# yhsong0804/P-NTFields

Measured on AMD Instinct MI355X. Metric: (start,goal) tau+grad-tau evals/sec at batch=1M, Gibson 3D, higher is better.
Workload: dtype f32; 1 GPU; gibson_multi_env_tau_grad (C3/C4 shape: 1048576 pairs/GPU, 10 envs, per-pair env id, dim 3); pairs_per_gpu=1048576, global_batch=1048576, envs=10, grad_mode=exact, allgather_outputs=False, parallelism=dp1, rccl_world_size=1

## Files before the change

p-ntfields_amd/csrc/pntf_wide.h:

```cpp
#pragma once
#include "pntf_field.h"
#include "pntf_stamp.h"

namespace pntf {

typedef float f32x16 __attribute__((ext_vector_type(16)));

__device__ __forceinline__ f32x16 mfma32(float a, float b, f32x16 c) {
  return __builtin_amdgcn_mfma_f32_32x32x2f32(a, b, c, 0, 0, 0);
}
__device__ __forceinline__ f32x16 zero16() {
  f32x16 z;
#pragma unroll
  for (int r = 0; r < 16; ++r) z[r] = 0.f;
  return z;
}

constexpr int WNL = 6;
typedef __bf16 wbf16x8 __attribute__((ext_vector_type(8)));
typedef __bf16 wbf16x2 __attribute__((ext_vector_type(2)));
typedef float wf32x2 __attribute__((ext_vector_type(2)));
__device__ __forceinline__ void wx6_split(const f32x16& v, int b, wbf16x8 (&s)[3]) {
#pragma unroll
  for (int i = 0; i < 4; ++i) {
    wf32x2 x = {v[8 * b + 2 * i], v[8 * b + 2 * i + 1]};
    const wbf16x2 p0 = __builtin_convertvector(x, wbf16x2);
#ifdef PNTF_ABL_NOSPLIT
    s[0][2 * i] = s[1][2 * i] = s[2][2 * i] = p0[0];
    s[0][2 * i + 1] = s[1][2 * i + 1] = s[2][2 * i + 1] = p0[1];
    continue;
#endif
#if PNTF_X6_DOT
    const wf32x2 r1 = x6_resid(x, p0);
    const wbf16x2 p1 = __builtin_convertvector(r1, wbf16x2);
    const wf32x2 r2 = x6_resid(r1, p1);
#else
    const wf32x2 r1 = x - __builtin_convertvector(p0, wf32x2);
    const wbf16x2 p1 = __builtin_convertvector(r1, wbf16x2);
    const wf32x2 r2 = r1 - __builtin_convertvector(p1, wf32x2);
#endif
    const wbf16x2 p2 = __builtin_convertvector(r2, wbf16x2);
    s[0][2 * i] = p0[0]; s[0][2 * i + 1] = p0[1];
    s[1][2 * i] = p1[0]; s[1][2 * i + 1] = p1[1];
    s[2][2 * i] = p2[0]; s[2][2 * i + 1] = p2[1];
  }
}
__device__ __forceinline__ f32x16 wx6_mma(const f32x4& w0, const f32x4& w1, const f32x4& w2,
                                          const wbf16x8 (&x)[3], f32x16 acc) {
  const wbf16x8 a0 = __builtin_bit_cast(wbf16x8, w0), a1 = __builtin_bit_cast(wbf16x8, w1),
                a2 = __builtin_bit_cast(wbf16x8, w2);
  acc = __builtin_amdgcn_mfma_f32_32x32x16_bf16(a2, x[0], acc, 0, 0, 0);
  acc = __builtin_amdgcn_mfma_f32_32x32x16_bf16(a1, x[1], acc, 0, 0, 0);
  acc = __builtin_amdgcn_mfma_f32_32x32x16_bf16(a0, x[2], acc, 0, 0, 0);
  acc = __builtin_amdgcn_mfma_f32_32x32x16_bf16(a1, x[0], acc, 0, 0, 0);
  acc = __builtin_amdgcn_mfma_f32_32x32x16_bf16(a0, x[1], acc, 0, 0, 0);
  return __builtin_amdgcn_mfma_f32_32x32x16_bf16(a0, x[0], acc, 0, 0, 0);
}
constexpr float WKAPPA = WIDE_KAPPA;
constexpr float WKAPPA_INV = 0.0693147180559945309f;
__device__ __forceinline__ SpSig wsp_sig(float y) {
#ifdef PNTF_ABL_CHEAPACT
  return SpSig{fmaxf(y, 0.f) * 0.5f + 0.01f, 0.5f};
#endif
  const float t = __builtin_amdgcn_exp2f(-fabsf(y));
  const float u = 1.f + t;
  const float r = __builtin_amdgcn_rcpf(u);
  const bool pos = y >= 0.f;
  SpSig o;
  o.sp = (pos ? y : 0.f) + __builtin_amdgcn_logf(u);
  o.sg = pos ? r : t * r;
  return o;
}

__device__ __forceinline__ constexpr int wrow(int r, int h) {
  return (r & 3) + 8 * (r >> 2) + 4 * h;
}

struct WScratch {
  Rsrc r;
};
__device__ __forceinline__ WScratch make_wscratch(float* p) {
  return WScratch{make_rsrc(p, p ? WSCRATCH_FLOATS_PER_WAVE * 4 : 0)};
}

typedef __attribute__((address_space(3))) f32x4 wlds_f4;
constexpr int WL_G3 = 0, WL_S0 = 4, WL_TILES = 8;
typedef __attribute__((address_space(3))) float wlds_f;
struct WLds {
  wlds_f4* p;
  const wlds_f* hw;
};
__device__ __forceinline__ void lstore(WLds l, int t, const f32x16& v) {
#pragma unroll
  for (int q = 0; q < 4; ++q)
    l.p[(t * 4 + q) * 64] = f32x4{v[4 * q], v[4 * q + 1], v[4 * q + 2], v[4 * q + 3]};
}
__device__ __forceinline__ f32x16 lload(WLds l, int t) {
  f32x16 v;
#pragma unroll
  for (int q = 0; q < 4; ++q) {
    const f32x4 p = l.p[(t * 4 + q) * 64];
#pragma unroll
    for (int s = 0; s < 4; ++s) v[4 * q + s] = p[s];
  }
  return v;
}

constexpr int WF = (OFF_WIDE + OFF_FWD) * 4;
constexpr int WB = (OFF_WIDE + OFF_BWD) * 4;
constexpr int WBC = (OFF_WIDE + W_OFF_BCOL) * 4;
constexpr int WHW = (OFF_WIDE + W_OFF_G4W) * 4;
constexpr int WG4B = (OFF_WIDE + W_OFF_G4B) * 4;

constexpr int wx6_base(int wide_base) { return OFF_X6 * 4 + (wide_base - OFF_WIDE * 4) / 2 * 3; }
struct WHead {
  int base;
  __device__ int operator()(int j, int l) const { return wx6_base(base) + (j * 6 + l) * 1024; }
};
struct WE0Head {
  __device__ int operator()(int j, int l) const {
    return wx6_base(WF + OFF_E0 * 4) + (j * 6 + l) * 1024;
  }
};
__device__ __forceinline__ WHead wbwd_head() { return WHead{WB + OFF_G3 * 4}; }
struct WFoldHead {
  __device__ int operator()(int j, int l) const {
    const int o = j / 8, kt = (j / 2) % 4, half = j % 2;
    return WB + OFF_E0 * 4 + ((((o + 4 * half) * 4 + kt) * 4 + l) * 1024);
  }
};
struct WFoldXHead {
  __device__ int operator()(int j, int l) const {
    return wx6_base(WB + OFF_E0 * 4) + (j * 6 + l) * 1024;
  }
};
template <class F>
constexpr int wnext_nl() {
  return std::is_same<F, WFoldHead>::value ? 4 : WNL;
}

template <int OT>
struct BiasCols {
  f32x4 v[(OT + 3) / 4];
  __device__ __forceinline__ void load(Rsrc W, int lane, int plain_off) {
#pragma unroll
    for (int g = 0; g < (OT + 3) / 4; ++g)
      v[g] = bload(W, lane * 16, WBC + ((plain_off / 128 + g) * 64) * 16);
  }
  __device__ __forceinline__ float operator()(int ot) const { return v[ot / 4][ot % 4]; }
};

__device__ __forceinline__ f32x4 wbw_load(const float* p) {
#ifdef PNTF_ABL_NOBW
  float v = 1e-3f * (float)(reinterpret_cast<uintptr_t>(p) & 255);
  asm volatile("v_mov_b32 %0, %0" : "+v"(v));
  return f32x4{v, v + 1e-4f, v + 2e-4f, v + 3e-4f};
#else
  return ld4(p);
#endif
}
template <bool BL>
struct WBt {
  __device__ __forceinline__ f32x4 load(const PairIO& io, int i) const {
    return wbw_load(io.Bw + i);
  }
};
template <>
struct WBt<true> {
  const wlds_f* t;
  __device__ __forceinline__ f32x4 load(const PairIO&, int i) const {
#ifdef PNTF_ABL_NOBW
    return wbw_load(reinterpret_cast<const float*>(static_cast<uintptr_t>(i)));
#else
    return *reinterpret_cast<const wlds_f4*>(t + i);
#endif
  }
};

__device__ __forceinline__ f32x4 whw_load(const WLds& wl, int t, int u, int h) {
#ifdef PNTF_ABL_NOHW
  float v = 1e-3f * (float)((t * 4 + u + h) & 255);
  asm volatile("v_mov_b32 %0, %0" : "+v"(v));
  return f32x4{v, v + 1e-4f, v + 2e-4f, v + 3e-4f};
#else
  return *reinterpret_cast<const wlds_f4*>(wl.hw + 32 * t + 8 * u + 4 * h);
#endif
}

template <int DIM, class BT>
__device__ __forceinline__ void wfourier_q(const PairIO& io, const BT& bt, int kt, int h,
                                           f32x16 (&q)[2]) {
#pragma unroll
  for (int c = 0; c < 2; ++c) q[c] = zero16();
#pragma unroll
  for (int d = 0; d < DIM; ++d)
#pragma unroll
    for (int u = 0; u < 4; ++u) {
      f32x4 b = bt.load(io, d * H + 32 * kt + 8 * u + 4 * h);
#pragma unroll
      for (int c = 0; c < 2; ++c)
#pragma unroll
        for (int s = 0; s < 4; ++s) q[c][4 * u + s] = fmaf(io.x[c][d], TWO_PI * b[s], q[c][4 * u + s]);
    }
}

template <int DIM, class BT, class AfterF>
__device__ __forceinline__ void wide_fold(Ring& ring, Rsrc W, const PairIO& io, BT bt,
                                          const f32x16 (&Y)[8], int lane, float (&ds)[DIM],
                                          float (&dg)[DIM], AfterF after) {
  const int h = lane >> 5;
  float acc[2][DIM];
#pragma unroll
  for (int d = 0; d < DIM; ++d) acc[0][d] = acc[1][d] = 0.f;
  f32x16 ph[2][2];
  run_steps<32, 4, wnext_nl<AfterF>(), SITE_FOLD>(
      ring, W, lane * 16, WFoldHead{}, after, [&](auto st, const f32x4 (&a)[4]) {
        constexpr int S = decltype(st)::value;
        constexpr int o = S / 8, kt = (S / 2) % 4, half = S % 2;
        if constexpr (kt == 0) {
#pragma unroll
          for (int c = 0; c < 2; ++c) ph[half][c] = zero16();
        }
#pragma unroll
        for (int u = 0; u < 4; ++u)
#pragma unroll
          for (int s = 0; s < 4; ++s)
#pragma unroll
            for (int c = 0; c < 2; ++c)
              ph[half][c] = mfma32(a[u][s], Y[c * 4 + kt][4 * u + s], ph[half][c]);
        if constexpr (kt == 3 && half == 1) {
#pragma unroll
          for (int u = 0; u < 4; ++u) {
            f32x4 bw[DIM];
#pragma unroll
            for (int d = 0; d < DIM; ++d) bw[d] = TWO_PI * bt.load(io, d * H + 32 * o + 8 * u + 4 * h);
#pragma unroll
            for (int c = 0; c < 2; ++c)
#pragma unroll
              for (int s = 0; s < 4; ++s) {
                float q = 0.f;
#pragma unroll
                for (int d = 0; d < DIM; ++d) q = fmaf(io.x[c][d], bw[d][s], q);
                float sn, cs;
                sincos_fast(q, sn, cs);
                const int r = 4 * u + s;
                float gg = ph[0][c][r] * cs - ph[1][c][r] * sn;
#pragma unroll
                for (int d = 0; d < DIM; ++d) acc[c][d] = fmaf(bw[d][s], gg, acc[c][d]);
              }
          }
        }
      });
#pragma unroll
  for (int d = 0; d < DIM; ++d) {
    ds[d] = acc[0][d] + __shfl_xor(acc[0][d], 32);
    dg[d] = acc[1][d] + __shfl_xor(acc[1][d], 32);
  }
}

template <class L>
struct XSched {
  static constexpr int STEPS = L::OT * L::KT;
  static constexpr int E(int j) { return STEPS - L::OT + 1 + j / L::CPS; }
  static constexpr int P(int j) { return E(j) - L::PDS; }
};
template <class L, int S>
__device__ __forceinline__ void xdue(L& ly) {
  if constexpr (L::NCH > 0) {
    static_for<0, L::NCH>([&](auto jj) {
      constexpr int j = decltype(jj)::value;
      if constexpr (L::PF && XSched<L>::P(j) == S) ly.prefetch(j);
    });
    static_for<0, L::NCH>([&](auto jj) {
      constexpr int j = decltype(jj)::value;
      if constexpr (XSched<L>::E(j) == S) ly.chunk(j);
    });
  }
}
template <class L>
struct XPend {
  L& ly;
  template <class ST>
  __device__ __forceinline__ void operator()(ST) const {
    xdue<L, XSched<L>::STEPS + ST::value>(ly);
  }
};
template <class L>
__device__ __forceinline__ void xflush(L& ly) {
  if constexpr (L::NCH > 0) {
    constexpr int S0 = XSched<L>::STEPS, S1 = XSched<L>::E(L::NCH - 1) + 1;
    if constexpr (S1 > S0)
      static_for<S0, S1>([&](auto ss) { xdue<L, decltype(ss)::value>(ly); });
  }
}

__device__ __forceinline__ void xagpr(f32x16& t) { asm("" : "+a"(t)); }

template <int OT, int KT, int NC, int SITE, class L, class PreF, class NextF>
__device__ __forceinline__ void xlayer(Ring& ring, Rsrc W, int wbase, f32x16 (&in)[8],
                                       int lane, L& ly, PreF pre, NextF naddr) {
  static_assert(NC * KT <= 8 && NC * OT <= 8, "bank size");
  static_assert(L::OT == OT && L::KT == KT && L::NC == NC, "layer object shape");
  constexpr int STEPS = OT * KT;
  wbf16x8 xs[NC][2][3];
  run_steps<STEPS, WNL, wnext_nl<NextF>(), SITE>(
      ring, W, lane * 16, WHead{wbase}, naddr, [&](auto st, const f32x4 (&a)[WNL]) {
        constexpr int S = decltype(st)::value;
        constexpr int kt = S / OT, ot = S % OT;
        pre(st);
        if constexpr (ot == 0) {
#pragma unroll
          for (int c = 0; c < NC; ++c)
#pragma unroll
            for (int b = 0; b < 2; ++b) wx6_split(in[c * KT + kt], b, xs[c][b]);
        }
        if constexpr (kt == 0) ly.init(ot);
#pragma unroll
        for (int b = 0; b < 2; ++b)
#pragma unroll
          for (int c = 0; c < NC; ++c)
            ly.out[c * OT + ot] = wx6_mma(a[3 * b], a[3 * b + 1], a[3 * b + 2], xs[c][b],
                                          ly.out[c * OT + ot]);
#pragma unroll
        for (int c = 0; c < NC; ++c) xagpr(ly.out[c * OT + ot]);
#pragma unroll
        for (int t = 0; t < 8; ++t) {
          xagpr(in[t]);
          xagpr(ly.out[t]);
        }
        xdue<L, S>(ly);
      });
}

template <int OT_, int KT_, int NC_, bool RES, bool SAVE, bool IN_LDS = false, bool ACT0 = false>
struct XFwdAct {
  static constexpr int OT = OT_, KT = KT_, NC = NC_, CPS = NC_, NCH = NC_ * OT_ * 4, PDS = 0;
  static constexpr bool PF = false;
  f32x16 (&out)[8];
  WScratch sc;
  int sc0, lane;
  BiasCols<OT_> bc;
  WLds wl;
  float cm;
  __device__ __forceinline__ void init(int ot) {
#pragma unroll
    for (int c = 0; c < NC; ++c)
      out[c * OT + ot] = mfma32(bc(ot), 1.f, RES ? out[c * OT + ot] : zero16());
  }
  __device__ __forceinline__ void prefetch(int) {}
  __device__ __forceinline__ void chunk(int j) {
    const int t = j / (4 * NC), c = (j / 4) % NC, q = j % 4;
    f32x4 g;
#pragma unroll
    for (int s = 0; s < 4; ++s) {
      const SpSig v = wsp_sig(out[c * OT + t][4 * q + s]);
      out[c * OT + t][4 * q + s] = v.sp;
      g[s] = ACT0 ? fmaf(cm, __builtin_amdgcn_rcpf(2.f - v.sg) - v.sg, v.sg) : v.sg;
    }
    if constexpr (SAVE && IN_LDS) wl.p[((sc0 + c * OT + t) * 4 + q) * 64] = g;
    else if constexpr (SAVE) bstore<AUX_NT>(sc.r, g, lane * 16, (sc0 + c * OT + t) * 4096 + q * 1024);
  }
};
template <int OT_, int KT_, int NC_>
struct XFwdLin {
  static constexpr int OT = OT_, KT = KT_, NC = NC_, CPS = 1, NCH = 0, PDS = 0;
  static constexpr bool PF = false;
  f32x16 (&out)[8];
  BiasCols<OT_> bc;
  __device__ __forceinline__ void init(int ot) {
#pragma unroll
    for (int c = 0; c < NC; ++c) out[c * OT + ot] = mfma32(bc(ot), 1.f, zero16());
  }
  __device__ __forceinline__ void prefetch(int) {}
  __device__ __forceinline__ void chunk(int) {}
};
template <int OT_, int KT_, int NC_, bool RES, bool MUL>
struct XBwd {
  static constexpr int OT = OT_, KT = KT_, NC = NC_, CPS = NC_, NCH = MUL ? NC_ * OT_ * 4 : 0;
  static constexpr int PDS = 3, NSLOT = CPS * (PDS + 1);
  static constexpr bool PF = MUL;
  f32x16 (&out)[8];
  WScratch sc;
  int mul0, lane;
  f32x4 sg[NSLOT];
  __device__ __forceinline__ void init(int ot) {
    if constexpr (!RES) {
#pragma unroll
      for (int c = 0; c < NC; ++c) out[c * OT + ot] = zero16();
    }
  }
  __device__ __forceinline__ void prefetch(int j) {
    const int t = j / (4 * NC), c = (j / 4) % NC, q = j % 4;
    sg[j % NSLOT] = __builtin_bit_cast(
        f32x4, __builtin_amdgcn_raw_buffer_load_b128(sc.r, lane * 16,
                                                     (mul0 + c * OT + t) * 4096 + q * 1024,
                                                     AUX_LOAD));
  }
  __device__ __forceinline__ void chunk(int j) {
    const int t = j / (4 * NC), c = (j / 4) % NC, q = j % 4;
#pragma unroll
    for (int s = 0; s < 4; ++s) out[c * OT + t][4 * q + s] *= sg[j % NSLOT][s];
  }
};

template <class BT>
constexpr bool xfold() { return std::is_same<BT, WBt<true>>::value; }

template <int DIM, class BT, class AfterF>
__device__ __forceinline__ void wide_fold_x(Ring& ring, Rsrc W, const PairIO& io, BT bt,
                                            f32x16 (&X)[8], f32x16 (&Y)[8], int lane,
                                            float (&ds)[DIM], float (&dg)[DIM], AfterF after) {
  const int h = lane >> 5;
  float acc[2][DIM];
#pragma unroll
  for (int d = 0; d < DIM; ++d) acc[0][d] = acc[1][d] = 0.f;
  wbf16x8 xs[2][2][3];
  run_steps<32, WNL, wnext_nl<AfterF>(), SITE_FOLD>(
      ring, W, lane * 16, WFoldXHead{}, after, [&](auto st, const f32x4 (&a)[WNL]) {
        constexpr int S = decltype(st)::value;
        constexpr int p = S / 16, kt = (S / 4) % 4, otl = S % 4;
        if constexpr (otl == 0) {
#pragma unroll
          for (int c = 0; c < 2; ++c)
#pragma unroll
            for (int b = 0; b < 2; ++b) wx6_split(Y[c * 4 + kt], b, xs[c][b]);
        }
        if constexpr (kt == 0) {
#pragma unroll
          for (int c = 0; c < 2; ++c) X[c * 4 + otl] = zero16();
        }
#pragma unroll
        for (int b = 0; b < 2; ++b)
#pragma unroll
          for (int c = 0; c < 2; ++c)
            X[c * 4 + otl] = wx6_mma(a[3 * b], a[3 * b + 1], a[3 * b + 2], xs[c][b], X[c * 4 + otl]);
#pragma unroll
        for (int c = 0; c < 2; ++c) xagpr(X[c * 4 + otl]);
#pragma unroll
        for (int t = 0; t < 8; ++t) xagpr(Y[t]);
        if constexpr (kt == 3 && otl == 3) {
#pragma unroll
          for (int ol = 0; ol < 2; ++ol) {
            const int o = 2 * p + ol;
#pragma unroll
            for (int u = 0; u < 4; ++u) {
              f32x4 bw[DIM];
#pragma unroll
              for (int d = 0; d < DIM; ++d)
                bw[d] = TWO_PI * bt.load(io, d * H + 32 * o + 8 * u + 4 * h);
#pragma unroll
              for (int c = 0; c < 2; ++c)
#pragma unroll
                for (int s = 0; s < 4; ++s) {
                  float q = 0.f;
#pragma unroll
                  for (int d = 0; d < DIM; ++d) q = fmaf(io.x[c][d], bw[d][s], q);
                  float sn, cs;
                  sincos_fast(q, sn, cs);
                  const int r = 4 * u + s;
                  const float gg = X[c * 4 + 2 * ol][r] * cs - X[c * 4 + 2 * ol + 1][r] * sn;
#pragma unroll
                  for (int d = 0; d < DIM; ++d) acc[c][d] = fmaf(bw[d][s], gg, acc[c][d]);
                }
            }
          }
        }
      });
#pragma unroll
  for (int d = 0; d < DIM; ++d) {
    ds[d] = acc[0][d] + __shfl_xor(acc[0][d], 32);
    dg[d] = acc[1][d] + __shfl_xor(acc[1][d], 32);
  }
}

template <int DIM, bool GRAD, class BT, class AfterF>
__device__ __forceinline__ float wide_forward_x(Ring& ring, Rsrc W, const PairIO& io, BT bt,
                                                f32x16 (&X)[8], f32x16 (&Y)[8], WScratch sc,
                                                WLds wl, int compat, int lane, AfterF after) {
  const int h = lane >> 5;
  XFwdAct<4, 8, 2, false, GRAD, false, true> e0{X, sc, WT_E0, lane, {}, wl, compat ? 1.f : 0.f};
  e0.bc.load(W, lane, B_E0);
  XFwdAct<4, 4, 2, false, GRAD> a0{Y, sc, WT_EBLK, lane, {}, wl, 0.f};
  {
    f32x16 q[2], sn[2];
    wbf16x8 xs[2][2][3];
    wfourier_q<DIM>(io, bt, 0, h, q);
    run_steps<32, WNL, WNL, SITE_FWD_E0>(
        ring, W, lane * 16, WE0Head{}, WHead{WF + OFF_EBLK * 4},
        [&](auto st, const f32x4 (&a)[WNL]) {
          constexpr int S = decltype(st)::value;
          constexpr int kt = S / 4, ot = S % 4;
          if constexpr (ot == 0 && kt < 4) {
#pragma unroll
            for (int c = 0; c < 2; ++c)
#pragma unroll
              for (int r = 0; r < 16; ++r) {
                float x0, x1;
                sincos_fast(q[c][r], x0, x1);
                sn[c][r] = x0;
                Y[c * 4 + kt][r] = x1;
              }
          }
          if constexpr (ot == 0) {
#pragma unroll
            for (int c = 0; c < 2; ++c)
#pragma unroll
              for (int b = 0; b < 2; ++b)
                wx6_split(kt < 4 ? sn[c] : Y[c * 4 + (kt & 3)], b, xs[c][b]);
          }
          if constexpr (kt == 0) e0.init(ot);
#pragma unroll
          for (int b = 0; b < 2; ++b)
#pragma unroll
            for (int c = 0; c < 2; ++c)
              X[c * 4 + ot] = wx6_mma(a[3 * b], a[3 * b + 1], a[3 * b + 2], xs[c][b], X[c * 4 + ot]);
#pragma unroll
          for (int c = 0; c < 2; ++c) xagpr(X[c * 4 + ot]);
#pragma unroll
          for (int t = 0; t < 8; ++t) {
            xagpr(X[t]);
            if (kt >= 4 || t % 4 < kt) xagpr(Y[t]);
          }
          if constexpr (ot == 3 && kt < 3) wfourier_q<DIM>(io, bt, kt + 1, h, q);
          if constexpr (S == 16) a0.bc.load(W, lane, B_EBLK);
          xdue<decltype(e0), S>(e0);
        });
  }

  const int WE = WF + OFF_EBLK * 4;
  {
    XFwdAct<4, 4, 2, true, GRAD> b0{X, sc, WT_EBLK + 8, lane, {}, wl, 0.f};
    XFwdAct<4, 4, 2, false, GRAD> a1{Y, sc, WT_EBLK + 16, lane, {}, wl, 0.f};
    XFwdAct<4, 4, 2, true, GRAD> b1{X, sc, WT_EBLK + 24, lane, {}, wl, 0.f};
    XFwdLin<4, 4, 2> e3{Y, {}};
    xlayer<4, 4, 2, SITE_FWD_ENC>(ring, W, WE, X, lane, a0,
                                  both(XPend<decltype(e0)>{e0},
                                       at<0>([&] { b0.bc.load(W, lane, B_EBLK + 128); })),
                                  WHead{WE + SZ_E * 4});
    xlayer<4, 4, 2, SITE_FWD_ENC>(ring, W, WE + SZ_E * 4, Y, lane, b0,
                                  both(XPend<decltype(a0)>{a0},
                                       at<0>([&] { a1.bc.load(W, lane, B_EBLK + 256); })),
                                  WHead{WE + 2 * SZ_E * 4});
    xlayer<4, 4, 2, SITE_FWD_ENC>(ring, W, WE + 2 * SZ_E * 4, X, lane, a1,
                                  both(XPend<decltype(b0)>{b0},
                                       at<0>([&] { b1.bc.load(W, lane, B_EBLK + 384); })),
                                  WHead{WE + 3 * SZ_E * 4});
    xlayer<4, 4, 2, SITE_FWD_ENC>(ring, W, WE + 3 * SZ_E * 4, Y, lane, b1,
                                  both(XPend<decltype(a1)>{a1},
                                       at<0>([&] { e3.bc.load(W, lane, B_E3); })),
                                  WHead{WF + OFF_E3 * 4});
    xlayer<4, 4, 2, SITE_FWD_ENC>(ring, W, WF + OFF_E3 * 4, X, lane, e3, XPend<decltype(b1)>{b1},
                                  WHead{WF + OFF_GBLK * 4});
  }

#pragma unroll
  for (int t = 0; t < 4; ++t) {
    f32x16 s0;
#pragma unroll
    for (int r = 0; r < 16; ++r) {
      float zs = Y[t][r], zg = Y[4 + t][r];
      float d = zs - zg;
      float e = __builtin_amdgcn_exp2f(-fabsf(d));
      float cc = __builtin_amdgcn_logf(1.f + e);
      X[t][r] = fmaxf(zs, zg) + cc;
      X[4 + t][r] = fminf(zs, zg) - cc;
      float rr = __builtin_amdgcn_rcpf(1.f + e);
      s0[r] = (d >= 0.f) ? rr : e * rr;
    }
    if (GRAD) lstore(wl, WL_S0 + t, s0);
  }

  XFwdAct<8, 8, 1, false, GRAD> ga{Y, sc, WT_GBLK, lane, {}, wl, 0.f};
  XFwdAct<8, 8, 1, true, GRAD> gb{X, sc, WT_GBLK + 8, lane, {}, wl, 0.f};
  ga.bc.load(W, lane, B_GBLK);
  xlayer<8, 8, 1, SITE_FWD_GEN>(ring, W, WF + OFF_GBLK * 4, X, lane, ga,
                                at<0>([&] { gb.bc.load(W, lane, B_GBLK + 256); }),
                                WHead{WF + (OFF_GBLK + SZ_G) * 4});
#pragma unroll 1
  for (int i = 0; i < 2; ++i) {
    const int wb = opaque(WF + (OFF_GBLK + (2 * i + 1) * SZ_G) * 4);
    const int wa = opaque(WF + (OFF_GBLK + (2 * i + 2) * SZ_G) * 4);
    const int wn = opaque(WF + (OFF_GBLK + (2 * i + 3) * SZ_G) * 4);
    const int ba = opaque(B_GBLK + (2 * i + 2) * 256);
    gb.sc0 = opaque(WT_GBLK + 16 * i + 8);
    xlayer<8, 8, 1, SITE_FWD_GEN>(ring, W, wb, Y, lane, gb,
                                  both(XPend<decltype(ga)>{ga},
                                       at<0>([&] { ga.bc.load(W, lane, ba); })),
                                  WHead{wa});
    ga.sc0 = opaque(WT_GBLK + 16 * i + 16);
    xlayer<8, 8, 1, SITE_FWD_GEN>(ring, W, wa, X, lane, ga,
                                  both(XPend<decltype(gb)>{gb},
                                       at<0>([&] { gb.bc.load(W, lane, ba + 256); })),
                                  WHead{wn});
  }
  XFwdAct<4, 8, 1, false, GRAD, true> g3{Y, sc, WL_G3, lane, {}, wl, 0.f};
  gb.sc0 = WT_GBLK + 16 * 2 + 8;
  xlayer<8, 8, 1, SITE_FWD_GEN>(ring, W, WF + (OFF_GBLK + 5 * SZ_G) * 4, Y, lane, gb,
                                both(XPend<decltype(ga)>{ga},
                                     at<0>([&] { g3.bc.load(W, lane, B_G3); })),
                                WHead{WF + OFF_G3 * 4});
  xlayer<4, 8, 1, SITE_FWD_GEN>(ring, W, WF + OFF_G3 * 4, X, lane, g3, XPend<decltype(gb)>{gb},
                                after);
  xflush(g3);
  float part = 0.f;
#pragma unroll
  for (int t = 0; t < 4; ++t)
#pragma unroll
    for (int u = 0; u < 4; ++u) {
      f32x4 w = whw_load(wl, t, u, h);
#pragma unroll
      for (int s = 0; s < 4; ++s) part = fmaf(w[s], Y[t][4 * u + s], part);
    }
  part += __shfl_xor(part, 32);
  const float y4 = fmaf(part, WKAPPA_INV, bload(W, 0, WG4B)[0]);
  return __builtin_amdgcn_rcpf(1.f + __builtin_amdgcn_exp2f(-0.144269504088896341f * y4));
}

template <int DIM, class BT, class AfterF>
__device__ __forceinline__ void wide_backward_x(Ring& ring, Rsrc W, const PairIO& io, BT bt,
                                                float tau, f32x16 (&X)[8], f32x16 (&Y)[8],
                                                WScratch sc, WLds wl, int lane,
                                                float (&ds)[DIM], float (&dg)[DIM],
                                                AfterF after) {
  const int h = lane >> 5;
  const float dd = 0.1f * tau * (1.f - tau);
#pragma unroll
  for (int t = 0; t < 4; ++t) {
    f32x16 s3 = lload(wl, WL_G3 + t);
#pragma unroll
    for (int u = 0; u < 4; ++u) {
      f32x4 w = whw_load(wl, t, u, h);
#pragma unroll
      for (int s = 0; s < 4; ++s) Y[t][4 * u + s] = (dd * w[s]) * s3[4 * u + s];
    }
  }
  XBwd<8, 4, 1, false, true> l3{X, sc, WT_GBLK + 16 * 2 + 8, lane, {}};
  xlayer<8, 4, 1, SITE_BWD_GEN>(ring, W, WB + OFF_G3 * 4, Y, lane, l3, NoPre{},
                                WHead{WB + (OFF_GBLK + 5 * SZ_G) * 4});
  XBwd<8, 8, 1, false, true> lb{Y, sc, WT_GBLK + 16 * 2, lane, {}};
  XBwd<8, 8, 1, true, true> la{X, sc, 0, lane, {}};
  xlayer<8, 8, 1, SITE_BWD_GEN>(ring, W, WB + (OFF_GBLK + 5 * SZ_G) * 4, X, lane, lb,
                                XPend<decltype(l3)>{l3}, WHead{WB + (OFF_GBLK + 4 * SZ_G) * 4});
#pragma unroll 1
  for (int i = 2; i >= 1; --i) {
    const int wa = opaque(WB + (OFF_GBLK + (2 * i) * SZ_G) * 4);
    const int wb = opaque(WB + (OFF_GBLK + (2 * i - 1) * SZ_G) * 4);
    const int wn = opaque(WB + (OFF_GBLK + (2 * i - 2) * SZ_G) * 4);
    la.mul0 = opaque(WT_GBLK + 16 * (i - 1) + 8);
    xlayer<8, 8, 1, SITE_BWD_GEN>(ring, W, wa, Y, lane, la, XPend<decltype(lb)>{lb}, WHead{wb});
    lb.mul0 = opaque(WT_GBLK + 16 * (i - 1));
    xlayer<8, 8, 1, SITE_BWD_GEN>(ring, W, wb, X, lane, lb, XPend<decltype(la)>{la}, WHead{wn});
  }
  {
    XBwd<8, 8, 1, true, false> l0{X, sc, 0, lane, {}};
    xlayer<8, 8, 1, SITE_BWD_GEN>(ring, W, WB + OFF_GBLK * 4, Y, lane, l0,
                                  XPend<decltype(lb)>{lb}, WHead{WB + OFF_E3 * 4});
  }
#pragma unroll
  for (int t = 0; t < 4; ++t) {
    f32x16 s0 = lload(wl, WL_S0 + t);
    f32x16 s1 = 1.f - s0;
    f32x16 dM = X[t], dm = X[4 + t];
    X[t] = s0 * dM + s1 * dm;
    X[4 + t] = s1 * dM + s0 * dm;
  }
  const int WE = WB + OFF_EBLK * 4;
  {
    XBwd<4, 4, 2, false, true> e3{Y, sc, WT_EBLK + 24, lane, {}};
    XBwd<4, 4, 2, false, true> b1{X, sc, WT_EBLK + 16, lane, {}};
    XBwd<4, 4, 2, true, true> a1{Y, sc, WT_EBLK + 8, lane, {}};
    XBwd<4, 4, 2, false, true> b0{X, sc, WT_EBLK, lane, {}};
    XBwd<4, 4, 2, true, true> a0{Y, sc, WT_E0, lane, {}};
    xlayer<4, 4, 2, SITE_BWD_ENC>(ring, W, WB + OFF_E3 * 4, X, lane, e3, NoPre{},
                                  WHead{WE + 3 * SZ_E * 4});
    xlayer<4, 4, 2, SITE_BWD_ENC>(ring, W, WE + 3 * SZ_E * 4, Y, lane, b1, XPend<decltype(e3)>{e3},
                                  WHead{WE + 2 * SZ_E * 4});
    xlayer<4, 4, 2, SITE_BWD_ENC>(ring, W, WE + 2 * SZ_E * 4, X, lane, a1, XPend<decltype(b1)>{b1},
                                  WHead{WE + 1 * SZ_E * 4});
    xlayer<4, 4, 2, SITE_BWD_ENC>(ring, W, WE + 1 * SZ_E * 4, Y, lane, b0, XPend<decltype(a1)>{a1},
                                  WHead{WE});
    if constexpr (xfold<BT>())
      xlayer<4, 4, 2, SITE_BWD_ENC>(ring, W, WE, X, lane, a0, XPend<decltype(b0)>{b0},
                                    WFoldXHead{});
    else
      xlayer<4, 4, 2, SITE_BWD_ENC>(ring, W, WE, X, lane, a0, XPend<decltype(b0)>{b0},
                                    WFoldHead{});
    xflush(a0);
  }
  if constexpr (xfold<BT>()) wide_fold_x<DIM>(ring, W, io, bt, X, Y, lane, ds, dg, after);
  else wide_fold<DIM>(ring, W, io, bt, Y, lane, ds, dg, after);
}

template <int DIM, int KIND, bool BL>
__global__ __launch_bounds__(256, 1) void wide_field_kernel(FieldArgs a) {
  PNTF_CLOCK_SCOPE;
  constexpr bool GRAD = KIND != K_TAU && KIND != K_TRAVEL;
  const int lane = threadIdx.x & 63;
  const int slot = blockIdx.x * WAVES + __builtin_amdgcn_readfirstlane(threadIdx.x >> 6);
  const int nslots = gridDim.x * WAVES;
  const int ntiles = (int)((a.n + WTILE - 1) / WTILE);
  const WScratch sc =
      make_wscratch(GRAD ? a.ws + (int64_t)slot * WSCRATCH_FLOATS_PER_WAVE : nullptr);
  const Rsrc W = make_rsrc(a.P, PACKED_TOTAL_X6 * 4);
  __shared__ f32x4 wsig[GRAD ? WAVES * WL_TILES * 4 * 64 : 1];
  __shared__ f32x4 whead[WAVES * H / 4];
  const int wv = __builtin_amdgcn_readfirstlane(threadIdx.x >> 6);
  const WLds wl{(wlds_f4*)wsig + (GRAD ? wv * (WL_TILES * 4 * 64) + lane : 0),
                (const wlds_f*)(whead + wv * (H / 4))};
  ((wlds_f*)(whead + wv * (H / 4)))[lane] = a.P[OFF_BIAS + B_G4W + lane];
  ((wlds_f*)(whead + wv * (H / 4)))[lane + 64] = a.P[OFF_BIAS + B_G4W + lane + 64];
  __shared__ f32x4 wbtab[BL ? WBL_FLOATS / 4 : 1];
  if constexpr (BL) {
    const int nb4 = a.n_env * (DIM * H / 4);
    for (int i = threadIdx.x; i < nb4; i += 256)
      wbtab[i] = *reinterpret_cast<const f32x4*>(a.Btab + 4 * i);
  }
  Ring ring;
  ring_fill<WNL>(ring, W, lane * 16, WE0Head{});
  if constexpr (BL) __syncthreads();
  for (int tile = slot; tile < ntiles; tile += nslots) {
    f32x16 X[8], Y[8];
    int v16 = lane * 16;
    asm volatile("" : "+v"(v16));
    const int64_t pair = (int64_t)(tile * WTILE + ((v16 >> 4) & 31));
    PairIO io;
    const bool ok = load_pair<DIM>(a.xp, a.Btab, a.env, a.n, a.n_env, pair, io);
    WBt<BL> bt;
    if constexpr (BL) bt.t = (const wlds_f*)wbtab + (io.Bw - a.Btab);
    float tau;
    if constexpr (GRAD)
      tau = wide_forward_x<DIM, true>(ring, W, io, bt, X, Y, sc, wl, a.compat, lane,
                                      wbwd_head());
    else
      tau = wide_forward_x<DIM, false>(ring, W, io, bt, X, Y, sc, wl, a.compat, lane,
                                       WE0Head{});
    float ds[DIM], dg[DIM];
    if constexpr (GRAD) {
      drain_stores();
      wide_backward_x<DIM>(ring, W, io, bt, tau, X, Y, sc, wl, lane, ds, dg, WE0Head{});
    }
    const bool store = lane < 32 && pair < a.n;
    store_field<DIM, KIND>(a, pair, ok, store, tau, io, ds, dg);
  }
}

#if defined(PNTF_UTIL)
__global__ void pack_wide_kernel(const float* __restrict__ src, int rows, int cols, int ld,
                                 int trans, float scale, float* __restrict__ dst) {
  int64_t o = (int64_t)blockIdx.x * blockDim.x + threadIdx.x;
  if (o >= (int64_t)rows * cols) return;
  int s = o & 3;
  int l = (o >> 2) & 63;
  int u = (o >> 8) & 3;
  int64_t rest = o >> 10;
  int KT = cols / 32;
  int kt = rest % KT;
  int ot = rest / KT;
  int n = 32 * ot + (l & 31);
  int k = 32 * kt + 8 * u + 4 * (l >> 5) + s;
  dst[o] = scale * (trans ? src[(int64_t)k * ld + n] : src[(int64_t)n * ld + k]);
}

__global__ void pack_x6_kernel(const float* __restrict__ wide, uint16_t* __restrict__ x6) {
  const int64_t t = (int64_t)blockIdx.x * blockDim.x + threadIdx.x;
  if (t >= (int64_t)(2 * SZ_DIR / 1024) * 2 * 64) return;
  const int lane = (int)(t & 63), b = (int)((t >> 6) & 1);
  const int gf = (int)(t >> 7);
  const int dir = gf >= SZ_DIR / 1024, f = gf * 1024 - dir * SZ_DIR;
  int m0, out, in;
  if (f < OFF_EBLK) { m0 = OFF_E0; out = 128; in = 256; }
  else if (f < OFF_GBLK) { m0 = OFF_EBLK + (f - OFF_EBLK) / SZ_E * SZ_E; out = in = 128; }
  else if (f < OFF_G3) { m0 = OFF_GBLK + (f - OFF_GBLK) / SZ_G * SZ_G; out = in = 256; }
  else { m0 = OFF_G3; out = 128; in = 256; }
  if (dir) { const int x = out; out = in; in = x; }
  const int OT = out / 32, KT = in / 32;
  const int j = (f - m0) / 1024, ot = j / KT, kt = j % KT;
  int64_t fr;
  if (dir && m0 == OFF_E0) {
    const int pp = (ot % 4) / 2, ol = ((ot % 4) % 2) * 2 + ot / 4;
    fr = ((int64_t)(gf - j) + (pp * KT + kt) * 4 + ol) * 6 + 3 * b;
  } else {
    fr = ((int64_t)(gf - j) + kt * OT + ot) * 6 + 3 * b;
  }
  const float* src = wide + (int64_t)gf * 1024;
  float v[8];
#pragma unroll
  for (int i = 0; i < 8; ++i) v[i] = src[((2 * b + (i >> 2)) * 64 + lane) * 4 + (i & 3)];
  f32x16 tile;
#pragma unroll
  for (int i = 0; i < 16; ++i) tile[i] = v[i & 7];
  wbf16x8 s[3];
  wx6_split(tile, 0, s);
#pragma unroll
  for (int p = 0; p < 3; ++p)
    *reinterpret_cast<wbf16x8*>(x6 + ((fr + p) * 64 + lane) * 8) = s[p];
}

__global__ void pack_wide_aux_kernel(const float* __restrict__ plain, float* __restrict__ wide) {
  const int o = blockIdx.x * blockDim.x + threadIdx.x;
  constexpr int NB = W_SZ_BCOL, NH = W_SZ_G4W;
  if (o < NB) {
    int s = o & 3, l = (o >> 2) & 63, g = o >> 8;
    wide[W_OFF_BCOL + o] = l < 32 ? WKAPPA * plain[128 * g + 32 * s + l] : 0.f;
  } else if (o < NB + NH) {
    int p = o - NB;
    int s = p & 3, l = (p >> 2) & 63, f = p >> 8;
    int t = f / 4, u = f % 4;
    wide[W_OFF_G4W + p] = plain[B_G4W + 32 * t + 8 * u + 4 * (l >> 5) + s];
  } else if (o < NB + NH + 4) {
    wide[W_OFF_G4B + (o - NB - NH)] = plain[B_G4B + (o - NB - NH)];
  }
}
#endif

}
```

Before: 70.78 million pairs/s.

## Defer layer epilogue into next layer's input consumption and prescale Fourier table by 2π

```diff
diff --git a/p-ntfields_amd/csrc/pntf_wide.h b/p-ntfields_amd/csrc/pntf_wide.h
--- a/p-ntfields_amd/csrc/pntf_wide.h
+++ b/p-ntfields_amd/csrc/pntf_wide.h
@@ -161,16 +161,16 @@
 }
 template <bool BL>
 struct WBt {
-  __device__ __forceinline__ f32x4 load(const PairIO& io, int i) const {
-    return wbw_load(io.Bw + i);
+  __device__ __forceinline__ f32x4 load2pi(const PairIO& io, int i) const {
+    return TWO_PI * wbw_load(io.Bw + i);
   }
 };
 template <>
 struct WBt<true> {
   const wlds_f* t;
-  __device__ __forceinline__ f32x4 load(const PairIO&, int i) const {
+  __device__ __forceinline__ f32x4 load2pi(const PairIO&, int i) const {
 #ifdef PNTF_ABL_NOBW
-    return wbw_load(reinterpret_cast<const float*>(static_cast<uintptr_t>(i)));
+    return TWO_PI * wbw_load(reinterpret_cast<const float*>(static_cast<uintptr_t>(i)));
 #else
     return *reinterpret_cast<const wlds_f4*>(t + i);
 #endif
@@ -196,11 +196,11 @@
   for (int d = 0; d < DIM; ++d)
 #pragma unroll
     for (int u = 0; u < 4; ++u) {
-      f32x4 b = bt.load(io, d * H + 32 * kt + 8 * u + 4 * h);
+      const f32x4 b = bt.load2pi(io, d * H + 32 * kt + 8 * u + 4 * h);
 #pragma unroll
       for (int c = 0; c < 2; ++c)
 #pragma unroll
-        for (int s = 0; s < 4; ++s) q[c][4 * u + s] = fmaf(io.x[c][d], TWO_PI * b[s], q[c][4 * u + s]);
+        for (int s = 0; s < 4; ++s) q[c][4 * u + s] = fmaf(io.x[c][d], b[s], q[c][4 * u + s]);
     }
 }
 
@@ -233,7 +233,7 @@
           for (int u = 0; u < 4; ++u) {
             f32x4 bw[DIM];
 #pragma unroll
-            for (int d = 0; d < DIM; ++d) bw[d] = TWO_PI * bt.load(io, d * H + 32 * o + 8 * u + 4 * h);
+            for (int d = 0; d < DIM; ++d) bw[d] = bt.load2pi(io, d * H + 32 * o + 8 * u + 4 * h);
 #pragma unroll
             for (int c = 0; c < 2; ++c)
 #pragma unroll
@@ -258,49 +258,32 @@
   }
 }
 
-template <class L>
-struct XSched {
-  static constexpr int STEPS = L::OT * L::KT;
-  static constexpr int E(int j) { return STEPS - L::OT + 1 + j / L::CPS; }
-  static constexpr int P(int j) { return E(j) - L::PDS; }
-};
-template <class L, int S>
-__device__ __forceinline__ void xdue(L& ly) {
-  if constexpr (L::NCH > 0) {
-    static_for<0, L::NCH>([&](auto jj) {
-      constexpr int j = decltype(jj)::value;
-      if constexpr (L::PF && XSched<L>::P(j) == S) ly.prefetch(j);
-    });
-    static_for<0, L::NCH>([&](auto jj) {
-      constexpr int j = decltype(jj)::value;
-      if constexpr (XSched<L>::E(j) == S) ly.chunk(j);
-    });
-  }
-}
-template <class L>
-struct XPend {
-  L& ly;
-  template <class ST>
-  __device__ __forceinline__ void operator()(ST) const {
-    xdue<L, XSched<L>::STEPS + ST::value>(ly);
-  }
+constexpr int XPDS = 3;
+struct XPlain {
+  static constexpr bool EPI = false, PF = false;
+  __device__ __forceinline__ void prefetch(int) {}
 };
 template <class L>
 __device__ __forceinline__ void xflush(L& ly) {
-  if constexpr (L::NCH > 0) {
-    constexpr int S0 = XSched<L>::STEPS, S1 = XSched<L>::E(L::NCH - 1) + 1;
-    if constexpr (S1 > S0)
-      static_for<S0, S1>([&](auto ss) { xdue<L, decltype(ss)::value>(ly); });
+  if constexpr (L::EPI) {
+    static_for<0, L::OT>([&](auto tt) {
+      constexpr int t = decltype(tt)::value;
+      if constexpr (L::PF && t > 0) ly.prefetch(t);
+#pragma unroll
+      for (int c = 0; c < L::NC; ++c) ly.template tile<true>(t, c);
+    });
   }
 }
 
 __device__ __forceinline__ void xagpr(f32x16& t) { asm("" : "+a"(t)); }
 
-template <int OT, int KT, int NC, int SITE, class L, class PreF, class NextF>
+template <int OT, int KT, int NC, int SITE, bool KEEP, class L, class P, class PreF, class NextF>
 __device__ __forceinline__ void xlayer(Ring& ring, Rsrc W, int wbase, f32x16 (&in)[8],
-                                       int lane, L& ly, PreF pre, NextF naddr) {
+                                       int lane, L& ly, P& pv, PreF pre, NextF naddr) {
   static_assert(NC * KT <= 8 && NC * OT <= 8, "bank size");
   static_assert(L::OT == OT && L::KT == KT && L::NC == NC, "layer object shape");
+  static_assert(XPDS < OT, "tile t - 1's sigma quads are used before tile t's are loaded");
+  if constexpr (P::EPI) static_assert(P::OT == KT && P::NC == NC, "previous layer's shape");
   constexpr int STEPS = OT * KT;
   wbf16x8 xs[NC][2][3];
   run_steps<STEPS, WNL, wnext_nl<NextF>(), SITE>(
@@ -308,11 +291,17 @@
         constexpr int S = decltype(st)::value;
         constexpr int kt = S / OT, ot = S % OT;
         pre(st);
+        if constexpr (P::PF && (S + XPDS) % OT == 0 && (S + XPDS) / OT < KT)
+          pv.prefetch((S + XPDS) / OT);
         if constexpr (ot == 0) {
 #pragma unroll
-          for (int c = 0; c < NC; ++c)
-#pragma unroll
-            for (int b = 0; b < 2; ++b) wx6_split(in[c * KT + kt], b, xs[c][b]);
+          for (int c = 0; c < NC; ++c) {
+            f32x16 v;
+            if constexpr (P::EPI) v = pv.template tile<KEEP>(kt, c);
+            else v = in[c * KT + kt];
+#pragma unroll
+            for (int b = 0; b < 2; ++b) wx6_split(v, b, xs[c][b]);
+          }
         }
         if constexpr (kt == 0) ly.init(ot);
 #pragma unroll
@@ -328,14 +317,14 @@
           xagpr(in[t]);
           xagpr(ly.out[t]);
         }
-        xdue<L, S>(ly);
+        if constexpr (L::PF && S == STEPS - XPDS) ly.prefetch(0);
       });
 }
 
 template <int OT_, int KT_, int NC_, bool RES, bool SAVE, bool IN_LDS = false, bool ACT0 = false>
 struct XFwdAct {
-  static constexpr int OT = OT_, KT = KT_, NC = NC_, CPS = NC_, NCH = NC_ * OT_ * 4, PDS = 0;
-  static constexpr bool PF = false;
+  static constexpr int OT = OT_, KT = KT_, NC = NC_;
+  static constexpr bool EPI = true, PF = false;
   f32x16 (&out)[8];
   WScratch sc;
   int sc0, lane;
@@ -348,23 +337,29 @@
       out[c * OT + ot] = mfma32(bc(ot), 1.f, RES ? out[c * OT + ot] : zero16());
   }
   __device__ __forceinline__ void prefetch(int) {}
-  __device__ __forceinline__ void chunk(int j) {
-    const int t = j / (4 * NC), c = (j / 4) % NC, q = j % 4;
-    f32x4 g;
-#pragma unroll
-    for (int s = 0; s < 4; ++s) {
-      const SpSig v = wsp_sig(out[c * OT + t][4 * q + s]);
-      out[c * OT + t][4 * q + s] = v.sp;
-      g[s] = ACT0 ? fmaf(cm, __builtin_amdgcn_rcpf(2.f - v.sg) - v.sg, v.sg) : v.sg;
+  template <bool KEEP>
+  __device__ __forceinline__ f32x16 tile(int t, int c) {
+    f32x16 v = out[c * OT + t];
+#pragma unroll
+    for (int q = 0; q < 4; ++q) {
+      f32x4 g;
+#pragma unroll
+      for (int s = 0; s < 4; ++s) {
+        const SpSig r = wsp_sig(v[4 * q + s]);
+        v[4 * q + s] = r.sp;
+        g[s] = ACT0 ? fmaf(cm, __builtin_amdgcn_rcpf(2.f - r.sg) - r.sg, r.sg) : r.sg;
+      }
+      if constexpr (SAVE && IN_LDS) wl.p[((sc0 + c * OT + t) * 4 + q) * 64] = g;
+      else if constexpr (SAVE) bstore<AUX_NT>(sc.r, g, lane * 16, (sc0 + c * OT + t) * 4096 + q * 1024);
     }
-    if constexpr (SAVE && IN_LDS) wl.p[((sc0 + c * OT + t) * 4 + q) * 64] = g;
-    else if constexpr (SAVE) bstore<AUX_NT>(sc.r, g, lane * 16, (sc0 + c * OT + t) * 4096 + q * 1024);
+    if constexpr (KEEP) out[c * OT + t] = v;
+    return v;
   }
 };
 template <int OT_, int KT_, int NC_>
 struct XFwdLin {
-  static constexpr int OT = OT_, KT = KT_, NC = NC_, CPS = 1, NCH = 0, PDS = 0;
-  static constexpr bool PF = false;
+  static constexpr int OT = OT_, KT = KT_, NC = NC_;
+  static constexpr bool EPI = false, PF = false;
   f32x16 (&out)[8];
   BiasCols<OT_> bc;
   __device__ __forceinline__ void init(int ot) {
@@ -372,44 +367,52 @@
     for (int c = 0; c < NC; ++c) out[c * OT + ot] = mfma32(bc(ot), 1.f, zero16());
   }
   __device__ __forceinline__ void prefetch(int) {}
-  __device__ __forceinline__ void chunk(int) {}
 };
 template <int OT_, int KT_, int NC_, bool RES, bool MUL>
 struct XBwd {
-  static constexpr int OT = OT_, KT = KT_, NC = NC_, CPS = NC_, NCH = MUL ? NC_ * OT_ * 4 : 0;
-  static constexpr int PDS = 3, NSLOT = CPS * (PDS + 1);
-  static constexpr bool PF = MUL;
+  static constexpr int OT = OT_, KT = KT_, NC = NC_;
+  static constexpr bool EPI = MUL, PF = MUL;
   f32x16 (&out)[8];
   WScratch sc;
   int mul0, lane;
-  f32x4 sg[NSLOT];
+  f32x4 sg[4 * NC_];
   __device__ __forceinline__ void init(int ot) {
     if constexpr (!RES) {
 #pragma unroll
       for (int c = 0; c < NC; ++c) out[c * OT + ot] = zero16();
     }
   }
-  __device__ __forceinline__ void prefetch(int j) {
-    const int t = j / (4 * NC), c = (j / 4) % NC, q = j % 4;
-    sg[j % NSLOT] = __builtin_bit_cast(
-        f32x4, __builtin_amdgcn_raw_buffer_load_b128(sc.r, lane * 16,
-                                                     (mul0 + c * OT + t) * 4096 + q * 1024,
-                                                     AUX_LOAD));
-  }
-  __device__ __forceinline__ void chunk(int j) {
-    const int t = j / (4 * NC), c = (j / 4) % NC, q = j % 4;
-#pragma unroll
-    for (int s = 0; s < 4; ++s) out[c * OT + t][4 * q + s] *= sg[j % NSLOT][s];
+  __device__ __forceinline__ void prefetch(int t) {
+#pragma unroll
+    for (int c = 0; c < NC; ++c)
+#pragma unroll
+      for (int q = 0; q < 4; ++q)
+        sg[c * 4 + q] = __builtin_bit_cast(
+            f32x4, __builtin_amdgcn_raw_buffer_load_b128(sc.r, lane * 16,
+                                                         (mul0 + c * OT + t) * 4096 + q * 1024,
+                                                         AUX_LOAD));
+  }
+  template <bool KEEP>
+  __device__ __forceinline__ f32x16 tile(int t, int c) {
+#pragma clang fp contract(off)
+    f32x16 v = out[c * OT + t];
+#pragma unroll
+    for (int q = 0; q < 4; ++q)
+#pragma unroll
+      for (int s = 0; s < 4; ++s) v[4 * q + s] *= sg[c * 4 + q][s];
+    if constexpr (KEEP) out[c * OT + t] = v;
+    return v;
   }
 };
 
 template <class BT>
 constexpr bool xfold() { return std::is_same<BT, WBt<true>>::value; }
 
-template <int DIM, class BT, class AfterF>
+template <int DIM, class BT, class P, class AfterF>
 __device__ __forceinline__ void wide_fold_x(Ring& ring, Rsrc W, const PairIO& io, BT bt,
-                                            f32x16 (&X)[8], f32x16 (&Y)[8], int lane,
+                                            f32x16 (&X)[8], f32x16 (&Y)[8], P& pv, int lane,
                                             float (&ds)[DIM], float (&dg)[DIM], AfterF after) {
+  static_assert(P::OT == 4 && P::NC == 2, "previous layer's shape");
   const int h = lane >> 5;
   float acc[2][DIM];
 #pragma unroll
@@ -419,11 +422,17 @@
       ring, W, lane * 16, WFoldXHead{}, after, [&](auto st, const f32x4 (&a)[WNL]) {
         constexpr int S = decltype(st)::value;
         constexpr int p = S / 16, kt = (S / 4) % 4, otl = S % 4;
+        if constexpr (P::PF && p == 0 && (S + XPDS) % 4 == 0 && (S + XPDS) / 4 < 4)
+          pv.prefetch((S + XPDS) / 4);
         if constexpr (otl == 0) {
 #pragma unroll
-          for (int c = 0; c < 2; ++c)
-#pragma unroll
-            for (int b = 0; b < 2; ++b) wx6_split(Y[c * 4 + kt], b, xs[c][b]);
+          for (int c = 0; c < 2; ++c) {
+            f32x16 v;
+            if constexpr (P::EPI && p == 0) v = pv.template tile<true>(kt, c);
+            else v = Y[c * 4 + kt];
+#pragma unroll
+            for (int b = 0; b < 2; ++b) wx6_split(v, b, xs[c][b]);
+          }
         }
         if constexpr (kt == 0) {
 #pragma unroll
@@ -447,7 +456,7 @@
               f32x4 bw[DIM];
 #pragma unroll
               for (int d = 0; d < DIM; ++d)
-                bw[d] = TWO_PI * bt.load(io, d * H + 32 * o + 8 * u + 4 * h);
+                bw[d] = bt.load2pi(io, d * H + 32 * o + 8 * u + 4 * h);
 #pragma unroll
               for (int c = 0; c < 2; ++c)
 #pragma unroll
@@ -523,7 +532,6 @@
           }
           if constexpr (ot == 3 && kt < 3) wfourier_q<DIM>(io, bt, kt + 1, h, q);
           if constexpr (S == 16) a0.bc.load(W, lane, B_EBLK);
-          xdue<decltype(e0), S>(e0);
         });
   }
 
@@ -533,24 +541,20 @@
     XFwdAct<4, 4, 2, false, GRAD> a1{Y, sc, WT_EBLK + 16, lane, {}, wl, 0.f};
     XFwdAct<4, 4, 2, true, GRAD> b1{X, sc, WT_EBLK + 24, lane, {}, wl, 0.f};
     XFwdLin<4, 4, 2> e3{Y, {}};
-    xlayer<4, 4, 2, SITE_FWD_ENC>(ring, W, WE, X, lane, a0,
-                                  both(XPend<decltype(e0)>{e0},
-                                       at<0>([&] { b0.bc.load(W, lane, B_EBLK + 128); })),
-                                  WHead{WE + SZ_E * 4});
-    xlayer<4, 4, 2, SITE_FWD_ENC>(ring, W, WE + SZ_E * 4, Y, lane, b0,
-                                  both(XPend<decltype(a0)>{a0},
-                                       at<0>([&] { a1.bc.load(W, lane, B_EBLK + 256); })),
-                                  WHead{WE + 2 * SZ_E * 4});
-    xlayer<4, 4, 2, SITE_FWD_ENC>(ring, W, WE + 2 * SZ_E * 4, X, lane, a1,
-                                  both(XPend<decltype(b0)>{b0},
-                                       at<0>([&] { b1.bc.load(W, lane, B_EBLK + 384); })),
-                                  WHead{WE + 3 * SZ_E * 4});
-    xlayer<4, 4, 2, SITE_FWD_ENC>(ring, W, WE + 3 * SZ_E * 4, Y, lane, b1,
-                                  both(XPend<decltype(a1)>{a1},
-                                       at<0>([&] { e3.bc.load(W, lane, B_E3); })),
-                                  WHead{WF + OFF_E3 * 4});
-    xlayer<4, 4, 2, SITE_FWD_ENC>(ring, W, WF + OFF_E3 * 4, X, lane, e3, XPend<decltype(b1)>{b1},
-                                  WHead{WF + OFF_GBLK * 4});
+    xlayer<4, 4, 2, SITE_FWD_ENC, true>(ring, W, WE, X, lane, a0, e0,
+                                        at<0>([&] { b0.bc.load(W, lane, B_EBLK + 128); }),
+                                        WHead{WE + SZ_E * 4});
+    xlayer<4, 4, 2, SITE_FWD_ENC, false>(ring, W, WE + SZ_E * 4, Y, lane, b0, a0,
+                                         at<0>([&] { a1.bc.load(W, lane, B_EBLK + 256); }),
+                                         WHead{WE + 2 * SZ_E * 4});
+    xlayer<4, 4, 2, SITE_FWD_ENC, true>(ring, W, WE + 2 * SZ_E * 4, X, lane, a1, b0,
+                                        at<0>([&] { b1.bc.load(W, lane, B_EBLK + 384); }),
+                                        WHead{WE + 3 * SZ_E * 4});
+    xlayer<4, 4, 2, SITE_FWD_ENC, false>(ring, W, WE + 3 * SZ_E * 4, Y, lane, b1, a1,
+                                         at<0>([&] { e3.bc.load(W, lane, B_E3); }),
+                                         WHead{WF + OFF_E3 * 4});
+    xlayer<4, 4, 2, SITE_FWD_ENC, false>(ring, W, WF + OFF_E3 * 4, X, lane, e3, b1, NoPre{},
+                                         WHead{WF + OFF_GBLK * 4});
   }
 
 #pragma unroll
@@ -573,9 +577,10 @@
   XFwdAct<8, 8, 1, false, GRAD> ga{Y, sc, WT_GBLK, lane, {}, wl, 0.f};
   XFwdAct<8, 8, 1, true, GRAD> gb{X, sc, WT_GBLK + 8, lane, {}, wl, 0.f};
   ga.bc.load(W, lane, B_GBLK);
-  xlayer<8, 8, 1, SITE_FWD_GEN>(ring, W, WF + OFF_GBLK * 4, X, lane, ga,
-                                at<0>([&] { gb.bc.load(W, lane, B_GBLK + 256); }),
-                                WHead{WF + (OFF_GBLK + SZ_G) * 4});
+  XPlain plain;
+  xlayer<8, 8, 1, SITE_FWD_GEN, true>(ring, W, WF + OFF_GBLK * 4, X, lane, ga, plain,
+                                      at<0>([&] { gb.bc.load(W, lane, B_GBLK + 256); }),
+                                      WHead{WF + (OFF_GBLK + SZ_G) * 4});
 #pragma unroll 1
   for (int i = 0; i < 2; ++i) {
     const int wb = opaque(WF + (OFF_GBLK + (2 * i + 1) * SZ_G) * 4);
@@ -583,24 +588,19 @@
     const int wn = opaque(WF + (OFF_GBLK + (2 * i + 3) * SZ_G) * 4);
     const int ba = opaque(B_GBLK + (2 * i + 2) * 256);
     gb.sc0 = opaque(WT_GBLK + 16 * i + 8);
-    xlayer<8, 8, 1, SITE_FWD_GEN>(ring, W, wb, Y, lane, gb,
-                                  both(XPend<decltype(ga)>{ga},
-                                       at<0>([&] { ga.bc.load(W, lane, ba); })),
-                                  WHead{wa});
+    xlayer<8, 8, 1, SITE_FWD_GEN, false>(ring, W, wb, Y, lane, gb, ga,
+                                         at<0>([&] { ga.bc.load(W, lane, ba); }), WHead{wa});
     ga.sc0 = opaque(WT_GBLK + 16 * i + 16);
-    xlayer<8, 8, 1, SITE_FWD_GEN>(ring, W, wa, X, lane, ga,
-                                  both(XPend<decltype(gb)>{gb},
-                                       at<0>([&] { gb.bc.load(W, lane, ba + 256); })),
-                                  WHead{wn});
+    xlayer<8, 8, 1, SITE_FWD_GEN, true>(ring, W, wa, X, lane, ga, gb,
+                                        at<0>([&] { gb.bc.load(W, lane, ba + 256); }),
+                                        WHead{wn});
   }
   XFwdAct<4, 8, 1, false, GRAD, true> g3{Y, sc, WL_G3, lane, {}, wl, 0.f};
   gb.sc0 = WT_GBLK + 16 * 2 + 8;
-  xlayer<8, 8, 1, SITE_FWD_GEN>(ring, W, WF + (OFF_GBLK + 5 * SZ_G) * 4, Y, lane, gb,
-                                both(XPend<decltype(ga)>{ga},
-                                     at<0>([&] { g3.bc.load(W, lane, B_G3); })),
-                                WHead{WF + OFF_G3 * 4});
-  xlayer<4, 8, 1, SITE_FWD_GEN>(ring, W, WF + OFF_G3 * 4, X, lane, g3, XPend<decltype(gb)>{gb},
-                                after);
+  xlayer<8, 8, 1, SITE_FWD_GEN, false>(ring, W, WF + (OFF_GBLK + 5 * SZ_G) * 4, Y, lane, gb, ga,
+                                       at<0>([&] { g3.bc.load(W, lane, B_G3); }),
+                                       WHead{WF + OFF_G3 * 4});
+  xlayer<4, 8, 1, SITE_FWD_GEN, false>(ring, W, WF + OFF_G3 * 4, X, lane, g3, gb, NoPre{}, after);
   xflush(g3);
   float part = 0.f;
 #pragma unroll
@@ -635,26 +635,27 @@
     }
   }
   XBwd<8, 4, 1, false, true> l3{X, sc, WT_GBLK + 16 * 2 + 8, lane, {}};
-  xlayer<8, 4, 1, SITE_BWD_GEN>(ring, W, WB + OFF_G3 * 4, Y, lane, l3, NoPre{},
-                                WHead{WB + (OFF_GBLK + 5 * SZ_G) * 4});
+  XPlain plain;
+  xlayer<8, 4, 1, SITE_BWD_GEN, true>(ring, W, WB + OFF_G3 * 4, Y, lane, l3, plain, NoPre{},
+                                      WHead{WB + (OFF_GBLK + 5 * SZ_G) * 4});
   XBwd<8, 8, 1, false, true> lb{Y, sc, WT_GBLK + 16 * 2, lane, {}};
   XBwd<8, 8, 1, true, true> la{X, sc, 0, lane, {}};
-  xlayer<8, 8, 1, SITE_BWD_GEN>(ring, W, WB + (OFF_GBLK + 5 * SZ_G) * 4, X, lane, lb,
-                                XPend<decltype(l3)>{l3}, WHead{WB + (OFF_GBLK + 4 * SZ_G) * 4});
+  xlayer<8, 8, 1, SITE_BWD_GEN, true>(ring, W, WB + (OFF_GBLK + 5 * SZ_G) * 4, X, lane, lb, l3,
+                                      NoPre{}, WHead{WB + (OFF_GBLK + 4 * SZ_G) * 4});
 #pragma unroll 1
   for (int i = 2; i >= 1; --i) {
     const int wa = opaque(WB + (OFF_GBLK + (2 * i) * SZ_G) * 4);
     const int wb = opaque(WB + (OFF_GBLK + (2 * i - 1) * SZ_G) * 4);
     const int wn = opaque(WB + (OFF_GBLK + (2 * i - 2) * SZ_G) * 4);
     la.mul0 = opaque(WT_GBLK + 16 * (i - 1) + 8);
-    xlayer<8, 8, 1, SITE_BWD_GEN>(ring, W, wa, Y, lane, la, XPend<decltype(lb)>{lb}, WHead{wb});
+    xlayer<8, 8, 1, SITE_BWD_GEN, false>(ring, W, wa, Y, lane, la, lb, NoPre{}, WHead{wb});
     lb.mul0 = opaque(WT_GBLK + 16 * (i - 1));
-    xlayer<8, 8, 1, SITE_BWD_GEN>(ring, W, wb, X, lane, lb, XPend<decltype(la)>{la}, WHead{wn});
+    xlayer<8, 8, 1, SITE_BWD_GEN, true>(ring, W, wb, X, lane, lb, la, NoPre{}, WHead{wn});
   }
   {
     XBwd<8, 8, 1, true, false> l0{X, sc, 0, lane, {}};
-    xlayer<8, 8, 1, SITE_BWD_GEN>(ring, W, WB + OFF_GBLK * 4, Y, lane, l0,
-                                  XPend<decltype(lb)>{lb}, WHead{WB + OFF_E3 * 4});
+    xlayer<8, 8, 1, SITE_BWD_GEN, false>(ring, W, WB + OFF_GBLK * 4, Y, lane, l0, lb, NoPre{},
+                                         WHead{WB + OFF_E3 * 4});
   }
 #pragma unroll
   for (int t = 0; t < 4; ++t) {
@@ -671,24 +672,23 @@
     XBwd<4, 4, 2, true, true> a1{Y, sc, WT_EBLK + 8, lane, {}};
     XBwd<4, 4, 2, false, true> b0{X, sc, WT_EBLK, lane, {}};
     XBwd<4, 4, 2, true, true> a0{Y, sc, WT_E0, lane, {}};
-    xlayer<4, 4, 2, SITE_BWD_ENC>(ring, W, WB + OFF_E3 * 4, X, lane, e3, NoPre{},
-                                  WHead{WE + 3 * SZ_E * 4});
-    xlayer<4, 4, 2, SITE_BWD_ENC>(ring, W, WE + 3 * SZ_E * 4, Y, lane, b1, XPend<decltype(e3)>{e3},
-                                  WHead{WE + 2 * SZ_E * 4});
-    xlayer<4, 4, 2, SITE_BWD_ENC>(ring, W, WE + 2 * SZ_E * 4, X, lane, a1, XPend<decltype(b1)>{b1},
-                                  WHead{WE + 1 * SZ_E * 4});
-    xlayer<4, 4, 2, SITE_BWD_ENC>(ring, W, WE + 1 * SZ_E * 4, Y, lane, b0, XPend<decltype(a1)>{a1},
-                                  WHead{WE});
-    if constexpr (xfold<BT>())
-      xlayer<4, 4, 2, SITE_BWD_ENC>(ring, W, WE, X, lane, a0, XPend<decltype(b0)>{b0},
-                                    WFoldXHead{});
-    else
-      xlayer<4, 4, 2, SITE_BWD_ENC>(ring, W, WE, X, lane, a0, XPend<decltype(b0)>{b0},
-                                    WFoldHead{});
-    xflush(a0);
-  }
-  if constexpr (xfold<BT>()) wide_fold_x<DIM>(ring, W, io, bt, X, Y, lane, ds, dg, after);
-  else wide_fold<DIM>(ring, W, io, bt, Y, lane, ds, dg, after);
+    xlayer<4, 4, 2, SITE_BWD_ENC, true>(ring, W, WB + OFF_E3 * 4, X, lane, e3, plain, NoPre{},
+                                        WHead{WE + 3 * SZ_E * 4});
+    xlayer<4, 4, 2, SITE_BWD_ENC, true>(ring, W, WE + 3 * SZ_E * 4, Y, lane, b1, e3, NoPre{},
+                                        WHead{WE + 2 * SZ_E * 4});
+    xlayer<4, 4, 2, SITE_BWD_ENC, false>(ring, W, WE + 2 * SZ_E * 4, X, lane, a1, b1, NoPre{},
+                                         WHead{WE + 1 * SZ_E * 4});
+    xlayer<4, 4, 2, SITE_BWD_ENC, true>(ring, W, WE + 1 * SZ_E * 4, Y, lane, b0, a1, NoPre{},
+                                        WHead{WE});
+    if constexpr (xfold<BT>()) {
+      xlayer<4, 4, 2, SITE_BWD_ENC, false>(ring, W, WE, X, lane, a0, b0, NoPre{}, WFoldXHead{});
+      wide_fold_x<DIM>(ring, W, io, bt, X, Y, a0, lane, ds, dg, after);
+    } else {
+      xlayer<4, 4, 2, SITE_BWD_ENC, false>(ring, W, WE, X, lane, a0, b0, NoPre{}, WFoldHead{});
+      xflush(a0);
+      wide_fold<DIM>(ring, W, io, bt, Y, lane, ds, dg, after);
+    }
+  }
 }
 
 template <int DIM, int KIND, bool BL>
@@ -713,7 +713,7 @@
   if constexpr (BL) {
     const int nb4 = a.n_env * (DIM * H / 4);
     for (int i = threadIdx.x; i < nb4; i += 256)
-      wbtab[i] = *reinterpret_cast<const f32x4*>(a.Btab + 4 * i);
+      wbtab[i] = TWO_PI * *reinterpret_cast<const f32x4*>(a.Btab + 4 * i);
   }
   Ring ring;
   ring_fill<WNL>(ring, W, lane * 16, WE0Head{});
```

Result: faster. 71.56 million pairs/s (median of 6 runs) (+1.1%).
